# Jackz915/PackPPI

Hardware: AMD Instinct MI355X
Metric: sampled residues/sec at 100 diffusion steps (higher is better)
Workload: dtype f32 (dense layers as split-f16: two f16 per operand, three f16 MFMAs per product, fp32 accumulate); 1 GPU; data/T1124_lig.pdb (L=739, 738 true residues), 1 complex per GPU; diffusion_steps=100, proximal=False, residues_per_gpu=738, residues_rank0=738, residues_total=738, mode=ode

## Files before the change

### packppi_amd/csrc/pp_api.hip

```cpp
#include <math.h>
#include <stdio.h>
#include <stdlib.h>
#include <string.h>

#include <new>
#include <string>
#include <vector>

#include "pp_internal.h"
#include "pp_topk_aten.h"
#include <algorithm>
#include <cstring>
#include <cmath>
#include <chrono>

static thread_local std::string g_err;
void pp_set_error(const std::string &msg) { g_err = msg; }

extern "C" const char *pp_last_error(void) { return g_err.c_str(); }
extern "C" int pp_version(void) { return 101; }
#ifndef PP_BUILD_ID
#define PP_BUILD_ID "unstamped-unstamped"
#endif
static const char g_build_id[] = "PP_BUILD_ID=" PP_BUILD_ID;
// ... 526 lines not shown
extern "C" void pp_ctx_destroy(pp_ctx *c) {
    if (!c) return;
    if (c->arena) {
        pp_plan *p = c->plan;
        std::lock_guard<std::mutex> g(p->pool_mutex);
        if (p->arena_pool.size() < 4) {
            p->arena_pool.push_back({c->arena, c->arena_bytes, c->last_stream});
        } else {
            (void)hipFree(c->arena);
        }
    }
    for (hipEvent_t e : c->prof_ev) (void)hipEventDestroy(e);
    delete c;
}

__global__ void k_fill_seg(int2 *__restrict__ seg, int N, int L) {
    const int n = blockIdx.x * blockDim.x + threadIdx.x;
    if (n < N) seg[n] = make_int2((n / L) * L, L);
}
__global__ void k_fill_seg_packed(int2 *__restrict__ seg, int N, const int32_t *__restrict__ off, int n_seg, int max_len) {
    const int n = blockIdx.x * blockDim.x + threadIdx.x;
    if (n >= N) return;
    int lo = 0, hi = n_seg - 1;
    while (lo < hi) {
        const int mid = (lo + hi + 1) >> 1;
        if (off[mid] <= n) lo = mid; else hi = mid - 1;
    }
    int start = off[lo], len = off[lo + 1] - off[lo];
    start = start < 0 ? 0 : (start > n ? n : start);
    len = len > max_len ? max_len : len;
// ... 78 lines not shown
        char *base = static_cast<char *>(c->arena);
        for (const Slot &sl : slots) { *sl.p = base; base += sl.bytes; }
    }
    if (st == PP_OK) {
        hipStream_t s_ = static_cast<hipStream_t>(stream);
        if (packed) hipLaunchKernelGGL(k_fill_seg_packed, dim3((c->N + 255) / 256), dim3(256), 0, s_, c->seg, c->N, seg_offsets, n_seg, c->L);
        else hipLaunchKernelGGL(k_fill_seg, dim3((c->N + 255) / 256), dim3(256), 0, s_, c->seg, c->N, c->L);
        if (hipGetLastError() != hipSuccess) { pp_set_error("segment table launch failed"); st = PP_ERR_HIP; }
    }
    if (st == PP_OK && hipMemsetAsync(c->sat, 0, 4 * sizeof(unsigned), static_cast<hipStream_t>(stream)) != hipSuccess) {
        pp_set_error("clearing the saturation word failed");
        st = PP_ERR_HIP;
    }
    if (net && st == PP_OK) flag_nonfinite(c, c->b.X, 42, 12, static_cast<hipStream_t>(stream));
    if (net && st == PP_OK) st = pp_launch_prepare(c, static_cast<hipStream_t>(stream));
    if (net && st == PP_OK) st = pp_launch_edge_static(c, static_cast<hipStream_t>(stream));
    if (st != PP_OK) { pp_ctx_destroy(c); return st; }
    *out = c;
    return PP_OK;
}

extern "C" pp_status pp_complex_prepare(pp_plan *plan, const pp_batch *b, void *stream, pp_ctx **out) {
    return prepare_impl(plan, b, nullptr, 0, 0, 0, stream, out);
}

extern "C" pp_status pp_complex_prepare_packed(pp_plan *plan, const pp_batch *b, const int32_t *seg_offsets, int n_seg,
                                               int min_len, int max_len, void *stream, pp_ctx **out) {
    if (!seg_offsets) FAIL(PP_ERR_INVALID, "pp_complex_prepare_packed: null segment offsets");
    return prepare_impl(plan, b, seg_offsets, n_seg, min_len, max_len, stream, out);
}
// ... 73 lines not shown
                             const StepParams *cur, const StepParams *next) {
    pp_status st;
    for (int l = 0; l < 3; l++) {
        if (l == 0 || !pp_edge_fused()) {
            prof_arm(c, 0);
            st = pp_launch_node_message(c, l, s);
            prof_disarm(c);
            if (st != PP_OK) return st;
        }
        if (l < 2) {
            prof_arm(c, 2);
            st = pp_launch_node_update(c, l, PP_NU_MID, chi, step, mode, noise, nullptr, nullptr, s);
            prof_disarm(c);
            if (st != PP_OK) return st;
            prof_arm(c, 1);
            st = pp_launch_edge_update(c, l, s);
            prof_disarm(c);
            if (st != PP_OK) return st;
        } else {
            prof_arm(c, 2);
            st = pp_launch_node_update(c, l, last_mode, chi, step, mode, noise, cur, last_mode == PP_NU_STEP ? next : nullptr, s);
            prof_disarm(c);
            if (st != PP_OK) return st;
        }
    }
    return PP_OK;
}

extern "C" pp_status pp_score(pp_ctx *c, const float *chi, float t, float *score, float *hV, void *stream) {
    if (c) c->last_stream = static_cast<hipStream_t>(stream);
    if (!c || !chi || !score) FAIL(PP_ERR_INVALID, "pp_score: null argument");
// ... 169 lines not shown
```

### packppi_amd/csrc/pp_edge.hip

```cpp
#include "pp_internal.h"

unsigned int pp_edge_range_hits(int) { return 0; }

typedef float f32x16 __attribute__((ext_vector_type(16)));
typedef float f32x4v __attribute__((ext_vector_type(4)));

#define ET 256
#define CH32 (128 * 32)
#define XBUF_FLOATS (4 * 4 * 64 * 4)
#define PARAM_FLOATS 1152

#define MFMA(a, b, c) __builtin_amdgcn_mfma_f32_32x32x2f32((a), (b), (c), 0, 0, 0)

struct EdgeArgs {
    int N, K;
    float inv_K;
    const float *rmask;
    const int32_t *eidx;
    const float *mask_att;
    const float *frames;
    const float *pts;
    const float *PA, *PC;
    const float *hE_in;
    float *hE_out;
// ... 288 lines not shown
    WSTAGE(C0 + 11 + 8 * (c) + 6, NCH, xbuf_get(xbuf, 2, lane, acc); mfma_tile32<false>(wslot, acc, out, lane))   \
    WSTAGE(C0 + 11 + 8 * (c) + 7, NCH, xbuf_get(xbuf, 3, lane, acc); mfma_tile32<false>(wslot, acc, out, lane))

template <int S, bool ST0, bool FUSE>
__global__ void __launch_bounds__(ET, PP_EU_WGS)
k_edge_update(EdgeArgs A) {
    extern __shared__ __attribute__((aligned(16))) float smem[];
    float *xbuf = smem + 4 * S * 1024, *prm = xbuf + XBUF_FLOATS;
    const int tid = threadIdx.x, lane = tid & 63;
    const int wave = __builtin_amdgcn_readfirstlane(tid >> 6);
    const int j = lane & 31, h = lane >> 5;
    const int n = blockIdx.x;
    const int K = A.K;
    const int jj = j < K ? j : K - 1;
    if (A.rmask[n] == 0.f) {
        if (j < K) {
            f32x4v z = {0.f, 0.f, 0.f, 0.f};
            float *orow = A.hE_out + ((size_t)n * K + j) * 128 + 32 * wave;
#pragma unroll
            for (int q = 0; q < 4; q++) *reinterpret_cast<f32x4v *>(orow + 8 * q + 4 * h) = z;
        }
        if constexpr (FUSE) {
            if (tid < 128) A.S[(size_t)n * 128 + tid] = 0.f;
            if (tid == 0) A.msum[n] = 0.f;
        }
        return;
    }
    constexpr int C0 = ST0 ? 0 : 4;
    constexpr int NEU = C0 + 43;
    constexpr int NCH = NEU + (FUSE ? 11 : 0);
    PROLOGUE_PIPE()
// ... 71 lines not shown
    else if (wave == 1) { _Pragma("unroll") for (int r = 0; r < 16; r++) out[r] += x[1][r]; }
    else if (wave == 2) { _Pragma("unroll") for (int r = 0; r < 16; r++) out[r] += x[2][r]; }
    else { _Pragma("unroll") for (int r = 0; r < 16; r++) out[r] += x[3][r]; }
    __syncthreads();
    xbuf_put(xbuf, wave, lane, out);
    __syncthreads();
#pragma unroll
    for (int t = 0; t < 4; t++) xbuf_get(xbuf, t, lane, x[t]);
    float mean3;
    const float rstd = ln_center(x, mean3);
#pragma unroll
    for (int r = 0; r < 16; r++) out[r] -= mean3;
    ln_affine_tile(out, rstd, A.g3 + 32 * wave, A.be3 + 32 * wave, h);
#pragma unroll
    for (int r = 0; r < 16; r++) out[r] *= me;
    store_tile(A.hE_out + ((size_t)n * K + jj) * 128 + 32 * wave, h, out);
    if constexpr (FUSE) {
        int o_pts = n * 48, o_fr = n * 12, o_pa = n * 128;
        int o_ptsj = nbr * 48, o_pc = nbr * 128;
        __syncthreads();
        xbuf_put(xbuf, wave, lane, out);
        asm volatile("" : "+s"(o_pts), "+s"(o_fr), "+s"(o_pa), "+v"(o_ptsj), "+v"(o_pc) : : "memory");
        edge_geometry(A.pts2 + o_pts, A.frames + o_fr, A.pts2 + o_ptsj, h, g);
        load_tile(A.PA2 + o_pa + 32 * wave, h, acc);
        add_tile(A.PC2 + o_pc + 32 * wave, h, acc);
        const float bmid = A.b_mid2[32 * wave + j];
        __builtin_amdgcn_sched_barrier(0);
        __syncthreads();
#pragma unroll
        for (int t = 0; t < 4; t++) xbuf_get(xbuf, t, lane, x[t]);
        WSTAGE(NEU + 0, NCH, mfma_tile32<false>(wslot, x[0], acc, lane))
// ... 111 lines not shown
}

void pp_edge_occupancy(int *node_msg, int *edge_upd) {
    edge_attrs();
    (void)hipOccupancyMaxActiveBlocksPerMultiprocessor(node_msg, reinterpret_cast<const void *>(k_node_message<PP_NM_SLOTS, false>), ET, NM_SMEM);
    (void)hipOccupancyMaxActiveBlocksPerMultiprocessor(edge_upd, reinterpret_cast<const void *>(k_edge_update<PP_EU_SLOTS, false, true>), ET, EU_SMEM);
}

#define EDGE_ATTR_CHECK()                                                                                   \
    if (!edge_attrs()) {                                                                                    \
        pp_set_error("hipFuncSetAttribute(MaxDynamicSharedMemorySize) failed for the edge kernels");        \
        return PP_ERR_HIP;                                                                                  \
    }

extern "C" int pp_edge_variant(void) { return 0; }
bool pp_edge_fused() { return true; }

pp_status pp_launch_edge_static(pp_ctx *c, hipStream_t s) {
    EDGE_ATTR_CHECK()
    EdgeArgs A = edge_args(c, 0, false);
    A.wstream = c->plan->static_stream;
    hipLaunchKernelGGL(k_edge_static<2>, dim3(c->N), dim3(ET), ST_SMEM, s, A);
    PP_HIP_CHECK(hipGetLastError());
    return PP_OK;
}

pp_status pp_launch_node_message(pp_ctx *c, int layer, hipStream_t s) {
    EDGE_ATTR_CHECK()
    EdgeArgs A = edge_args(c, layer, false);
    if (layer == 0) PP_LAUNCH(c, (k_node_message<PP_NM_SLOTS, true>), dim3(c->N), dim3(ET), NM_SMEM, s, A);
    else PP_LAUNCH(c, (k_node_message<PP_NM_SLOTS, false>), dim3(c->N), dim3(ET), NM_SMEM, s, A);
    PP_HIP_CHECK(hipGetLastError());
    return PP_OK;
}

pp_status pp_launch_edge_update(pp_ctx *c, int layer, hipStream_t s) {
    EDGE_ATTR_CHECK()
    if (layer < 0 || layer > 1) { pp_set_error("pp_launch_edge_update: layer must be 0 or 1"); return PP_ERR_INVALID; }
    EdgeArgs A = edge_args(c, layer, true);
    if (layer == 0) PP_LAUNCH(c, (k_edge_update<PP_EU_SLOTS, true, true>), dim3(c->N), dim3(ET), EU_SMEM, s, A);
    else PP_LAUNCH(c, (k_edge_update<PP_EU_SLOTS, false, true>), dim3(c->N), dim3(ET), EU_SMEM, s, A);
    PP_HIP_CHECK(hipGetLastError());
    return PP_OK;
}
```

### packppi_amd/csrc/pp_edge_f16.hip

```cpp
#include "pp_internal.h"

PP_RANGE_COUNTER
PP_RANGE_READER(pp_edge_range_hits)

typedef float f32x16 __attribute__((ext_vector_type(16)));
typedef float f32x4v __attribute__((ext_vector_type(4)));
typedef _Float16 h8 __attribute__((ext_vector_type(8)));

struct HT {
    h8 hi[2], lo[2];
};
typedef float f32x2v __attribute__((ext_vector_type(2)));
typedef _Float16 h2v __attribute__((ext_vector_type(2)));
typedef __fp16 fp16x2_t __attribute__((ext_vector_type(2)));
__device__ __forceinline__ h2v cvt2(f32x2v x) {
    const fp16x2_t r = __builtin_amdgcn_cvt_pkrtz(x[0], x[1]);
    return __builtin_bit_cast(h2v, r);
}
__device__ __forceinline__ f32x2v split_residual(h2v hh, f32x2v x) {
    const unsigned hp = __builtin_bit_cast(unsigned, hh);
    float d0, d1;
    asm("v_fma_mix_f32 %0, %1, -1.0, %2 op_sel_hi:[1,0,0]" : "=v"(d0) : "v"(hp), "v"(x[0]));
    asm("v_fma_mix_f32 %0, %1, -1.0, %2 op_sel:[1,0,0] op_sel_hi:[1,0,0]" : "=v"(d1) : "v"(hp), "v"(x[1]));
    return f32x2v{d0, d1};
// ... 51 lines not shown
    const float *hE_in;
    float *hE_out;
    float *S, *msum;
    const float *wstream;
    const float *params;
    const float *g3, *be3;
    const float *b_mid;
    const float *Z;
    const float *pts2, *PA2, *PC2, *b_mid2;
    float *Znm, *Zem;
    const float *ls_in, *ls_x1, *ls_out;
    unsigned *sat;
    float *dbg;
    int n_pairs;
    int mix_mode;
};
enum { P_BMID = 0, P_BOUT = 128, P_FOB = 256, P_G2 = 384, P_BE2 = 512, P_FIB = 640 };

#ifndef PP_WDEPTH
#define PP_WDEPTH 2
#endif
#ifndef PP_WDEPTH_R1
#define PP_WDEPTH_R1 2
#endif
#define WDEPTH_ (R == 1 ? PP_WDEPTH_R1 : PP_WDEPTH)
#if defined(PP_X_TS) && defined(PP_X_TS_FINE)
#define TSF(k) if constexpr ((k) >= PP_X_TS_FINE && (k) < PP_X_TS_FINE + 16) tsf[(k) - PP_X_TS_FINE] = (int)(__builtin_readcyclecounter() - ts0f);
#else
#define TSF(k)
#endif
// ... 447 lines not shown
        if (live[r]) {
            if (h == 0) A.S[(size_t)n[r] * 128 + 32 * wave + j] = s * A.inv_K;
            if (tid == 0) A.msum[n[r]] = ms * A.inv_K;
        }
    }
    if (pp_sat_hit(sat)) atomicOr(A.sat, 1u);
}

#ifndef PP_NM_WGS2
#define PP_NM_WGS2 3
#endif
template <int R, bool ST0>
__global__ void __launch_bounds__(ET, R == 1 ? PP_WGS : PP_NM_WGS2)
k_node_message(EdgeArgs A) {
    extern __shared__ __attribute__((aligned(16))) float smem[];
    node_message_body<R, ST0>(A, blockIdx.x * R, smem);
}

#define FFN_BIAS_FETCH(c) load_tile(A.params + P_FIB + 128 * (c) + 32 * wave, h, fib);
#define FFN_BLOCK(c)                                                                                         \
    _Pragma("unroll") for (int r = 0; r < R; r++) acc[r] = fib;                                              \
    if constexpr ((c) == 0) { RLAYER_OWN(C0 + 11 + 8 * (c), NCH, acc, x1buf, false, false) }                 \
    else { RLAYER_BUF(C0 + 11 + 8 * (c), NCH, acc, x1buf, false, true) }                                     \
    PUBLISH_OWN(true, acc, xbuf)                                                                             \
    if constexpr ((c) < 3) { FFN_BIAS_FETCH((c) + 1) }                                                       \
    RLAYER_OWN(C0 + 11 + 8 * (c) + 4, NCH, out, xbuf, false, false)

#ifdef PP_X_TS
#define TS(i) { tsv[i] = (int)(__builtin_readcyclecounter() - ts0); }
#else
#define TS(i)
#endif
template <int R, bool ST0, bool FUSE, bool LNS = false>
__device__ __forceinline__ void edge_update_body(const EdgeArgs &A, const int res0, float *smem) {
    float *const xbuf = smem, *const x1buf = smem + R * XBUF_FLOATS, *const stat = x1buf + R * XBUF_FLOATS,
                 *const prm = stat + R * STAT_FLOATS;
    const int tid = threadIdx.x, lane = tid & 63;
    const int wave = __builtin_amdgcn_readfirstlane(tid >> 6);
    const int j = lane & 31, h = lane >> 5;
    const int K = A.K;
    const int jj = j < K ? j : K - 1;
    unsigned sat = 0;
    GROUP_SETUP()
#pragma unroll
    for (int r = 0; r < R; r++)
        if (inr[r] && !live[r]) {
            if (j < K) {
                f32x4v z = {0.f, 0.f, 0.f, 0.f};
                float *orow = A.hE_out + ((size_t)n[r] * K + j) * 128 + 32 * wave;
#pragma unroll
                for (int q = 0; q < 4; q++) *reinterpret_cast<f32x4v *>(orow + 8 * q + 4 * h) = z;
            }
            if constexpr (FUSE) {
                if (tid < 128) A.S[(size_t)n[r] * 128 + tid] = 0.f;
                if (tid == 0) A.msum[n[r]] = 0.f;
            }
        }
    if (first < 0) return;
#pragma unroll
    for (int r = 0; r < R; r++)
        if (!live[r]) n[r] = first;
    constexpr int C0 = ST0 ? 0 : 4;
// ... 98 lines not shown
    FFN_BLOCK(3)
    TS(10)
#pragma unroll
    for (int r = 0; r < R; r++) ln_partial(out[r], stat + r * STAT_FLOATS, wave, j, h);
    __syncthreads();
    TS(11)
#pragma unroll
    for (int r = 0; r < R; r++) {
        float mean3;
        const float rstd = ln_merge(stat + r * STAT_FLOATS, j, mean3);
#pragma unroll
        for (int q = 0; q < 16; q++) out[r][q] -= mean3;
        ln_affine_tile(out[r], rstd, prm + PARAM_LDS + 32 * wave, prm + PARAM_LDS + 128 + 32 * wave, h);
#pragma unroll
        for (int q = 0; q < 16; q++) out[r][q] *= me[r];
        if (live[r]) store_tile(A.hE_out + ((size_t)n[r] * K + jj) * 128 + 32 * wave, h, out[r]);
    }
    TS(12)
    if constexpr (FUSE) {
        GeoI gi_[R];
        float pj2[R][3];
#pragma unroll
        for (int r = 0; r < R; r++) {
            asm volatile("" : "+v"(nbr[r]));
            geo_load_i(A.pts2 + (size_t)n[r] * 48, A.frames + (size_t)n[r] * 12, h, wave, gi_[r]);
            geo_load_j(A.pts2 + (size_t)nbr[r] * 48, h, wave, pj2[r]);
            load_tile(A.PA2 + (size_t)n[r] * 128 + 32 * wave, h, acc[r]);
        }
        __builtin_amdgcn_sched_barrier(0);
        PUBLISH_OPERAND(out, xbuf, A.ls_out)
        __builtin_amdgcn_sched_barrier(0);
// ... 52 lines not shown
    TS(17)
    if (A.dbg && tid == 0)
        for (int q = 0; q < 18; q++) A.dbg[(size_t)n[0] * 24 + q] = (float)tsv[q];
    if (A.dbg && tid == 0) A.dbg[(size_t)n[0] * 24 + 18] = (float)((ts0 >> 6) & 0xFFFFF);
#ifdef PP_X_TS_FINE
    if (A.dbg && tid == 0)
        for (int q = 0; q < 16; q++) A.dbg[(size_t)n[0] * 24 + q] = (float)tsf[q];
#endif
#endif
}

template <int R, bool ST0, bool FUSE, bool LNS = false>
__global__ void __launch_bounds__(ET, R == 1 ? PP_WGS : PP_WGS2)
k_edge_update(EdgeArgs A) {
    extern __shared__ __attribute__((aligned(16))) float smem[];
    edge_update_body<R, ST0, FUSE, LNS>(A, blockIdx.x * R, smem);
}

template <bool ST0, bool FUSE, bool LNS = false>
__global__ void __launch_bounds__(ET, 2)
k_edge_update_mix(EdgeArgs A) {
    extern __shared__ __attribute__((aligned(16))) float smem[];
    const int b = blockIdx.x;
    int pair = -1, single = -1;
    if (A.mix_mode == 2) {
        const int ns = gridDim.x - A.n_pairs;
        if (b < 2 * ns) { if (b & 1) single = b >> 1; else pair = b >> 1; }
        else pair = b - ns;
    } else if (A.mix_mode == 3) {
        const int ns = gridDim.x - A.n_pairs;
        if (b < ns) single = b; else pair = b - ns;
    } else {
        if (b < A.n_pairs) pair = b; else single = b - A.n_pairs;
    }
    if (pair >= 0) edge_update_body<2, ST0, FUSE, LNS>(A, 2 * pair, smem);
    else edge_update_body<1, ST0, FUSE, LNS>(A, 2 * A.n_pairs + single, smem);
}

template <bool ST0>
__global__ void __launch_bounds__(ET, 2)
k_node_message_mix(EdgeArgs A) {
    extern __shared__ __attribute__((aligned(16))) float smem[];
    const int b = blockIdx.x;
    const int ns = gridDim.x - A.n_pairs;
    if (b < ns) node_message_body<1, ST0>(A, 2 * A.n_pairs + b, smem);
    else node_message_body<2, ST0>(A, 2 * (b - ns), smem);
}

template <bool LNS>
__global__ void __launch_bounds__(ET, 1)
k_edge_static(EdgeArgs A) {
    extern __shared__ __attribute__((aligned(16))) float smem[];
    constexpr int R = 1;
    const int tid = threadIdx.x, lane = tid & 63;
    const int wave = __builtin_amdgcn_readfirstlane(tid >> 6);
    const int j = lane & 31, h = lane >> 5;
    const int n = blockIdx.x;
    const int K = A.K;
// ... 170 lines not shown
    PP_HIP_CHECK(hipGetLastError());
    return PP_OK;
}

static float *g_dbg = nullptr;
#ifdef PP_DIAG
extern "C" void pp_debug_set_dbg(float *p) { g_dbg = p; }
#endif
static EdgeArgs edge_args(pp_ctx *c, int layer, bool edge) {
    const pp_plan *p = c->plan;
    const LayerOff &o = p->off.layer[layer];
    EdgeArgs A;
    A.N = c->N; A.K = c->K; A.inv_K = 1.0f / (float)c->K;
    A.n_pairs = 0;
    A.mix_mode = 0;
    A.rmask = c->b.residue_mask;
    A.eidx = c->eidx; A.mask_att = c->mask_att; A.frames = c->frames;
    A.pts = edge ? c->ptsE : c->ptsN;
    A.PA = edge ? c->PAe : c->PAn;
    A.PC = edge ? c->PCe : c->PCn;
    A.hE_in = layer == 0 ? c->hE0 : c->hE;
    A.hE_out = c->hE;
    A.S = c->S; A.msum = c->msum;
    A.wstream = edge ? p->lt[layer].em_stream : p->lt[layer].nm_stream;
    A.params = p->lt[layer].em_params;
    A.g3 = p->w + o.norm_g[3]; A.be3 = p->w + o.norm_b[3];
    A.b_mid = p->w + o.nm_mid_b;
    A.Z = edge ? c->Zem : c->Znm;
    A.Znm = c->Znm; A.Zem = c->Zem;
    A.pts2 = c->ptsN; A.PA2 = c->PAn; A.PC2 = c->PCn;
// ... 89 lines not shown
    }
    if (g_forced_R >= 1 && g_forced_R <= PP_RMAX) return g_forced_R;
    return N > PP_WGS * g_num_cu ? 2 : 1;
}

static int g_mix = -1;
static bool use_mix(int N) {
    if (g_mix < 0) {
        const char *e = PP_GETENV("PP_EDGE_MIX");
        g_mix = e ? atoi(e) : 3;
    }
    if (g_forced_R >= 1 || !g_mix) return false;
    return N > 2 * g_num_cu && N <= 3 * g_num_cu;
}

void pp_edge_occupancy(int *node_msg, int *edge_upd) {
    edge_attrs();
    (void)hipOccupancyMaxActiveBlocksPerMultiprocessor(node_msg, reinterpret_cast<const void *>(nm_kernel_r(1, false)), ET, nm_smem(1));
    (void)hipOccupancyMaxActiveBlocksPerMultiprocessor(edge_upd, reinterpret_cast<const void *>(eu_kernel_r(1, false)), ET, eu_smem(1));
}

#define EDGE_ATTR_CHECK()                                                                                   \
    if (!edge_attrs()) {                                                                                    \
        pp_set_error("hipFuncSetAttribute(MaxDynamicSharedMemorySize) failed for the edge kernels");        \
        return PP_ERR_HIP;                                                                                  \
    }

pp_status pp_launch_edge_static(pp_ctx *c, hipStream_t s) {
    EDGE_ATTR_CHECK()
    EdgeArgs A = edge_args(c, 0, false);
// ... 3 lines not shown
    PP_HIP_CHECK(hipGetLastError());
    return PP_OK;
}

pp_status pp_launch_node_message(pp_ctx *c, int layer, hipStream_t s) {
    EDGE_ATTR_CHECK()
    EdgeArgs A = edge_args(c, layer, false);
    static const char *nm_env = PP_GETENV("PP_NM_R");
    static const int nm_R = nm_env ? atoi(nm_env) : 0;
    const int R = (nm_R >= 1 && nm_R <= PP_RMAX) ? nm_R : pick_R(c->N);
    static const char *nmix_env = PP_GETENV("PP_NM_MIX");
    static const bool nmix = !(nmix_env && atoi(nmix_env) == 0);
    if (nmix && !(nm_R >= 1 && nm_R <= PP_RMAX) && use_mix(c->N)) {
        A.n_pairs = (c->N + 2) / 3;
        const int singles = c->N - 2 * A.n_pairs > 0 ? c->N - 2 * A.n_pairs : 0;
        PP_LAUNCH(c, (layer == 0 ? k_node_message_mix<true> : k_node_message_mix<false>), dim3(A.n_pairs + singles), dim3(ET),
                  nm_smem(2), s, A);
        PP_HIP_CHECK(hipGetLastError());
        return PP_OK;
    }
    PP_LAUNCH(c, nm_kernel_r(R, layer == 0), dim3((c->N + R - 1) / R), dim3(ET), nm_smem(R), s, A);
    PP_HIP_CHECK(hipGetLastError());
    return PP_OK;
}

extern "C" int pp_edge_variant(void) { return 1; }
bool pp_edge_fused() { return PP_FUSED; }

pp_status pp_launch_edge_update(pp_ctx *c, int layer, hipStream_t s) {
    EDGE_ATTR_CHECK()
    if (layer < 0 || layer > 1) { pp_set_error("pp_launch_edge_update: layer must be 0 or 1"); return PP_ERR_INVALID; }
    EdgeArgs A = edge_args(c, layer, true);
    const int R = pick_R(c->N);
    const bool lns = c->plan->ln_scale != nullptr;
    if (lns && !PP_FUSED) { pp_set_error("pp_launch_edge_update: a plan with LayerNorm operand scales needs the fused build"); return PP_ERR_UNSUPPORTED; }
    if (use_mix(c->N)) {
        A.n_pairs = (c->N + 2) / 3;
        A.mix_mode = g_mix;
        const int singles = c->N - 2 * A.n_pairs > 0 ? c->N - 2 * A.n_pairs : 0;
        PP_LAUNCH(c, mix_kernel(layer == 0, lns), dim3(A.n_pairs + singles), dim3(ET), eu_smem(2) > eu_smem(1) ? eu_smem(2) : eu_smem(1), s, A);
        PP_HIP_CHECK(hipGetLastError());
        return PP_OK;
    }
    PP_LAUNCH(c, eu_kernel_r(R, layer == 0, lns), dim3((c->N + R - 1) / R), dim3(ET), eu_smem(R), s, A);
    PP_HIP_CHECK(hipGetLastError());
    return PP_OK;
}
```

### packppi_amd/csrc/pp_internal.h

```cpp
#pragma once
#include <hip/hip_runtime.h>
#include <hip/hip_ext.h>
#include <vector>
#include <mutex>
#include <stdint.h>
#include <string>

#include "../../include/packppi_hip.h"

#if defined(PP_LAB) && !defined(PP_DIAG)
#define PP_DIAG
#endif
#if !defined(PP_LAB) &&                                                                                                       \
    (defined(PP_X_TS) || defined(PP_X_TS_FINE) || defined(PP_X_NOWLOAD) || defined(PP_X_E_NOMFMA) || defined(PP_X_NOSAT) ||      \
     defined(PP_WDEPTH) || defined(PP_WDEPTH_R1) || defined(PP_NXB_R1) || defined(PP_WGS2) || defined(PP_WGS) ||                 \
     defined(PP_NM_WGS2) ||                                                                                                  \
     defined(PP_LDS_PAD) || defined(PP_NO_FUSE_NM) || defined(PP_NU_DEPTH))
#error "PP_X_* / tuning switches compile laboratory variants (most give wrong results): add -DPP_LAB and build a TAGGED library (python -m packppi_amd.build --tag NAME -DPP_LAB -DPP_X_...)"
#endif
#ifdef PP_DIAG
#define PP_GETENV(name) getenv(name)
#else
#define PP_GETENV(name) ((const char *)nullptr)
#endif
// ... 62 lines not shown
    float *side_extent;
    float *bounds_lower, *bounds_upper;
    float clash_tol;
    bool clash_params_set;
};

struct StepParams {
    float temb[16];
    float c_ode;
    float w;
    float c_drift;
    float c_diff;
    float pad[12];
};

struct pp_ctx {
    pp_plan *plan;
    pp_batch b;
    int B, L, K, N;
    bool packed = false;
    int2 *seg;
    int32_t *eidx;
    float *mask_att;
    float *frames;
    float *bbpos;
    float *hE0;
    float *Znm, *Zem;
    float *hE;
    float *hV;
    float *hV_alt;
    float *S;
    float *msum;
    float *ptsN, *PAn, *PCn;
    float *ptsE, *PAe, *PCe;
    float *score;
    float *chi_tmp;
    void *arena = nullptr;
// ... 100 lines not shown
    const float ang = sgn * acosf(pp_dot_t(n1, n2));
    return (ang != ang) ? 0.f : ang;
}
#endif

pp_status pp_launch_prepare(pp_ctx *c, hipStream_t s, const int64_t *E_idx = nullptr);
pp_status pp_launch_node_embed(pp_ctx *c, const float *chi, const StepParams &sp, hipStream_t s);
pp_status pp_launch_node_update(pp_ctx *c, int layer, int last_mode, float *chi, int step, int mode,
                                const float *noise, const StepParams *cur, const StepParams *next, hipStream_t s);
pp_status pp_launch_edge_static(pp_ctx *c, hipStream_t s);
#ifdef PP_EDGE_F16
pp_status pp_launch_edge_embed_f16(pp_ctx *c, hipStream_t s);
#endif
pp_status pp_launch_node_message(pp_ctx *c, int layer, hipStream_t s);
bool pp_edge_fused();
pp_status pp_launch_edge_update(pp_ctx *c, int layer, hipStream_t s);
pp_status pp_launch_atom14(pp_ctx *c, const float *chi, float *xyz, hipStream_t s);
pp_status pp_launch_clash(pp_ctx *c, const float *xyz, float *per_res, float *dchi, hipStream_t s, bool use_candidates = false);
pp_status pp_launch_proximal(pp_ctx *c, const float *chi, float lamda, int nsteps, float *traj,
                             float *chi_last, float *losses, hipStream_t s);

void pp_edge_occupancy(int *node_msg, int *edge_upd);

#define PP_NU_MID 0
#define PP_NU_SCORE 1
#define PP_NU_STEP 2
```

### packppi_amd/csrc/pp_node.hip

```cpp
#include <string.h>

#include "pp_internal.h"
#include <utility>

PP_RANGE_COUNTER
PP_RANGE_READER(pp_node_range_hits)

#define NT 512
#ifndef PP_NODE_GROUPS
#define PP_NODE_GROUPS 1
#endif
#define NG PP_NODE_GROUPS
#define NB (4 * NG)

struct NodeArgs {
    int N;
    const float *rmask;
    const int64_t *rtype;
    const float *bb_sincos;
    const float *sc_mask;
    const uint8_t *m1pi, *m2pi;
    const float *frames;
    const float *embT, *emb_b, *emb_g, *emb_beta;
    float *hV, *S, *msum;
// ... 258 lines not shown
struct NUpdArgs {
    int N;
    const float *rmask;
    const int64_t *rtype;
    const float *bb_sincos;
    const float *sc_mask;
    const uint8_t *m1pi, *m2pi;
    const float *frames;
    const float *embT;
    const float *wstream, *params;
    const float *hV;
    float *hV_out;
    const float *S, *msum;
    float *ptsN, *PAn, *PCn, *ptsE, *PAe, *PCe, *score;
    unsigned *sat;
};

template <bool LAST>
__device__ constexpr int nu_slot_waves(int s) {
    if (!LAST) return s < 52 ? 8 : 3;
    return s < 36 ? 8 : s < 40 ? 4 : s < 46 ? 1 : s < 55 ? 8 : 2;
}

template <int CL>
__device__ __forceinline__ int nu_phys_slot(int s, int q) {
    if constexpr (CL == 1) return s;
    constexpr int NPS = 16 / CL;
    return s < 36 ? s : s < 36 + NPS ? s + NPS * q : s + (16 - NPS);
}
template <bool LAST, int CL>
// ... 102 lines not shown
    _Pragma("unroll") for (int ks_ = 0; ks_ < 4; ks_++) ldB(HI, LO, r * NU_S128 + 8 * g, ks_, bh[ks_], bl[ks_]);
#define FOSTAGE(s)                                                                                   \
    NSTAGE(20 + (s), cH, {                                                                           \
        if constexpr ((s) + 1 < 16) ldB(sm.c_hi, sm.c_lo, r * NU_S512 + 8 * g, (s) + 1, fh[((s) + 1) & 1], fl[((s) + 1) & 1]); \
        mm3(AK, fh[(s) & 1], fl[(s) & 1], cH, cL);                                                   \
    })

template <int MODE, int NU_ND, int CL = 1>
__global__ void __launch_bounds__(512)
k_node_update(NUpdArgs A, float *chi, int step, int sde, const float *noise, int embed_next, StepScalars sp, TimeEmb te_next) {
    static_assert(CL == 1 || MODE == PP_NU_MID, "only the middle layers have a split form");
    constexpr int NU_NRING = NU_ND + 1;
    constexpr bool LAST = MODE != PP_NU_MID;
    constexpr int NSLOT = LAST ? PP_NU_SLOTS_LAST : PP_NU_SLOTS_MID;
    constexpr int NLOAD = MODE == PP_NU_SCORE ? 46 : CL > 1 ? 36 + 16 / CL + 4 : NSLOT;
    const int clq = CL > 1 ? (int)(blockIdx.x % CL) : 0;
    constexpr int NPAR = LAST ? NU_P_LAST_TOTAL : NU_P_MID_TOTAL;
    extern __shared__ __attribute__((aligned(16))) char smem_raw[];
    SmemU &sm = *reinterpret_cast<SmemU *>(smem_raw);
    const int tid = threadIdx.x, lane = tid & 63, wv = __builtin_amdgcn_readfirstlane(tid >> 6);
    const int r = lane & 15, g = lane >> 4, N = A.N, n0 = (int)(blockIdx.x / CL) * 16;
    const int n = n0 + r, nc = n < N ? n : N - 1;
    const bool live = n < N;
    const int fc = 16 * wv + 4 * g;
    const float *par = sm.par;

    const int srow = tid >> 5, scol = (tid & 31) * 4, sn = n0 + srow < N ? n0 + srow : N - 1;
    const nf4 s4 = *reinterpret_cast<const nf4 *>(A.S + (size_t)sn * 128 + scol);
    const nf4 hv4 = *reinterpret_cast<const nf4 *>(A.hV + (size_t)nc * 128 + fc);
    const float ms = A.msum[nc], rm = A.rmask[nc];
    const nf4 zero4i = {0.f, 0.f, 0.f, 0.f};
    float chi1 = 0.f, scm1 = 0.f, nz1 = 0.f, nz2 = 0.f;
    unsigned char m1raw = 0, m2raw = 0;
    int rt = 0;
    nf4 spv = zero4i;
    if constexpr (MODE == PP_NU_STEP) {
// ... 661 lines not shown
    A.rmask = c->b.residue_mask;
    A.rtype = c->b.residue_type;
    A.bb_sincos = c->b.BB_D_sincos;
    A.sc_mask = c->b.SC_D_mask;
    A.m1pi = c->b.chi_1pi_periodic_mask;
    A.m2pi = c->b.chi_2pi_periodic_mask;
    A.frames = c->frames;
    A.embT = p->node_emb_T;
    A.wstream = t.nu_stream;
    A.params = t.nu_params;
    A.hV = c->hV; A.hV_out = c->hV; A.S = c->S; A.msum = c->msum;
    A.ptsN = c->ptsN; A.PAn = c->PAn; A.PCn = c->PCn;
    A.ptsE = c->ptsE; A.PAe = c->PAe; A.PCe = c->PCe;
    A.score = c->score;
    A.sat = c->sat;
    int embed_next = (last_mode == PP_NU_STEP && embed_next_step) ? 1 : 0;
    const dim3 grid((c->N + 15) / 16), block(512);
    const int sde = mode == PP_MODE_SDE ? 1 : 0;
    StepScalars sp = {0.f, 0.f, 0.f, 0.f};
    TimeEmb te = {};
    if (cur) sp = {cur->c_ode, cur->w, cur->c_drift, cur->c_diff};
    if (next) memcpy(te.v, next->temb, sizeof(te.v));
#ifndef PP_EDGE_F16
    {
        static const bool f16_node = PP_GETENV("PP_NODE_F16") != nullptr;
        if (!f16_node) {
            const LayerOff &o = p->off.layer[layer];
            NodeArgs NA = make_args(c);
            UpdW W;
            W.outT = t.nm_out_T; W.out_b = p->w + o.nm_out_b;
// ... 16 lines not shown
            else
                PP_LAUNCH(c, k_node_update_valu<PP_NU_SCORE>, vgrid, vblock, sizeof(Smem), s, NA, W, chi, step, sde, noise, embed_next, pre0, sp, te);
            PP_HIP_CHECK(hipGetLastError());
            return PP_OK;
        }
    }
#endif
    const bool multi = (int)grid.x > g_nu_cus;
    static const char *split_env = PP_GETENV("PP_NU_SPLIT");
    static const int split_max = split_env ? atoi(split_env) : 4;
    const int tiles = (int)grid.x;
    const int cl = last_mode != PP_NU_MID ? 1 : (split_max >= 4 && 4 * tiles <= g_nu_cus) ? 4 : (split_max >= 2 && 2 * tiles <= g_nu_cus) ? 2 : 1;
    if (cl > 1) {
        A.hV_out = c->hV_alt;
        std::swap(c->hV, c->hV_alt);
        PP_LAUNCH(c, nu_kernel_split(cl), dim3(tiles * cl), block, sizeof(SmemU), s, A, chi, step, sde, noise, embed_next, sp, te);
        PP_HIP_CHECK(hipGetLastError());
        return PP_OK;
    }
    const nu_kernel_t kern = nu_kernel(last_mode == PP_NU_MID ? 0 : last_mode == PP_NU_STEP ? 1 : 2, multi);
    PP_LAUNCH(c, kern, grid, block, sizeof(SmemU), s, A, chi, step, sde, noise, embed_next, sp, te);
    PP_HIP_CHECK(hipGetLastError());
    return PP_OK;
}
```

Baseline: 61660 residues/s.

## Map residue blocks to XCDs for neighbour locality and skip dead hE store

Adds an XCD-aware block-to-work mapping so that contiguous residue ranges (and their mostly local kNN neighbours) are processed on the same XCD of the MI355X. The node-message, edge-update and node-update kernels all use it, with the aim of improving L2 hit rates for neighbour gathers. Separately, the last layer's edge update in STEP mode no longer writes hE_out, because that output is unused, which saves global stores. The remapping relies on round-robin dispatch of blocks to XCDs and can leave some blocks idle through early returns.

```diff
diff --git a/packppi_amd/csrc/pp_api.hip b/packppi_amd/csrc/pp_api.hip
--- a/packppi_amd/csrc/pp_api.hip
+++ b/packppi_amd/csrc/pp_api.hip
@@ -564,6 +564,19 @@
     delete c;
 }
 
+static void xcd_report(pp_ctx *c, hipStream_t s) {
+    std::vector<int32_t> e((size_t)c->N * c->K);
+    if (hipStreamSynchronize(s) != hipSuccess ||
+        hipMemcpy(e.data(), c->eidx, e.size() * sizeof(int32_t), hipMemcpyDeviceToHost) != hipSuccess) return;
+    std::vector<int> cls(c->N, 0);
+    for (int i = 0; i < 16; i++)
+        for (int r = pp_xcd_bnd(c->xmap, i); r < pp_xcd_bnd(c->xmap, i + 1) && r < c->N; r++) cls[r] = i & 7;
+    size_t same = 0;
+    for (size_t q = 0; q < e.size(); q++) same += (unsigned)e[q] < (unsigned)c->N && cls[q / c->K] == cls[e[q]];
+    fprintf(stderr, "[pp] XCD map: N %d, %d pairs + %d items of %d, %.1f %% of the %zu neighbour pairs on one XCD\n", c->N, c->xmap.P,
+            c->xmap.S, c->xmap.Rs, 100.0 * same / (double)e.size(), e.size());
+}
+
 __global__ void k_fill_seg(int2 *__restrict__ seg, int N, int L) {
     const int n = blockIdx.x * blockDim.x + threadIdx.x;
     if (n < N) seg[n] = make_int2((n / L) * L, L);
@@ -672,6 +685,8 @@
     }
     if (net && st == PP_OK) flag_nonfinite(c, c->b.X, 42, 12, static_cast<hipStream_t>(stream));
     if (net && st == PP_OK) st = pp_launch_prepare(c, static_cast<hipStream_t>(stream));
+    if (net) c->xmap = pp_edge_xcd_map(c->N);
+    if (net && st == PP_OK && c->xmap.on && PP_GETENV("PP_DEBUG")) xcd_report(c, static_cast<hipStream_t>(stream));
     if (net && st == PP_OK) st = pp_launch_edge_static(c, static_cast<hipStream_t>(stream));
     if (st != PP_OK) { pp_ctx_destroy(c); return st; }
     *out = c;
@@ -775,7 +790,7 @@
             prof_disarm(c);
             if (st != PP_OK) return st;
             prof_arm(c, 1);
-            st = pp_launch_edge_update(c, l, s);
+            st = pp_launch_edge_update(c, l, s, l == 0 || last_mode != PP_NU_STEP);
             prof_disarm(c);
             if (st != PP_OK) return st;
         } else {
diff --git a/packppi_amd/csrc/pp_edge.hip b/packppi_amd/csrc/pp_edge.hip
--- a/packppi_amd/csrc/pp_edge.hip
+++ b/packppi_amd/csrc/pp_edge.hip
@@ -326,7 +326,7 @@
     const int K = A.K;
     const int jj = j < K ? j : K - 1;
     if (A.rmask[n] == 0.f) {
-        if (j < K) {
+        if (j < K && A.hE_out) {
             f32x4v z = {0.f, 0.f, 0.f, 0.f};
             float *orow = A.hE_out + ((size_t)n * K + j) * 128 + 32 * wave;
 #pragma unroll
@@ -428,7 +428,7 @@
     ln_affine_tile(out, rstd, A.g3 + 32 * wave, A.be3 + 32 * wave, h);
 #pragma unroll
     for (int r = 0; r < 16; r++) out[r] *= me;
-    store_tile(A.hE_out + ((size_t)n * K + jj) * 128 + 32 * wave, h, out);
+    if (A.hE_out) store_tile(A.hE_out + ((size_t)n * K + jj) * 128 + 32 * wave, h, out);
     if constexpr (FUSE) {
         int o_pts = n * 48, o_fr = n * 12, o_pa = n * 128;
         int o_ptsj = nbr * 48, o_pc = nbr * 128;
@@ -570,6 +570,7 @@
     }
 
 extern "C" int pp_edge_variant(void) { return 0; }
+PPXcd pp_edge_xcd_map(int) { return PPXcd{}; }
 bool pp_edge_fused() { return true; }
 
 pp_status pp_launch_edge_static(pp_ctx *c, hipStream_t s) {
@@ -590,10 +591,11 @@
     return PP_OK;
 }
 
-pp_status pp_launch_edge_update(pp_ctx *c, int layer, hipStream_t s) {
+pp_status pp_launch_edge_update(pp_ctx *c, int layer, hipStream_t s, bool store_hE) {
     EDGE_ATTR_CHECK()
     if (layer < 0 || layer > 1) { pp_set_error("pp_launch_edge_update: layer must be 0 or 1"); return PP_ERR_INVALID; }
     EdgeArgs A = edge_args(c, layer, true);
+    if (!store_hE) A.hE_out = nullptr;
     if (layer == 0) PP_LAUNCH(c, (k_edge_update<PP_EU_SLOTS, true, true>), dim3(c->N), dim3(ET), EU_SMEM, s, A);
     else PP_LAUNCH(c, (k_edge_update<PP_EU_SLOTS, false, true>), dim3(c->N), dim3(ET), EU_SMEM, s, A);
     PP_HIP_CHECK(hipGetLastError());
diff --git a/packppi_amd/csrc/pp_edge_f16.hip b/packppi_amd/csrc/pp_edge_f16.hip
--- a/packppi_amd/csrc/pp_edge_f16.hip
+++ b/packppi_amd/csrc/pp_edge_f16.hip
@@ -89,6 +89,7 @@
     float *dbg;
     int n_pairs;
     int mix_mode;
+    PPXcd xm;
 };
 enum { P_BMID = 0, P_BOUT = 128, P_FOB = 256, P_G2 = 384, P_BE2 = 512, P_FIB = 640 };
 
@@ -566,7 +567,9 @@
 __global__ void __launch_bounds__(ET, R == 1 ? PP_WGS : PP_NM_WGS2)
 k_node_message(EdgeArgs A) {
     extern __shared__ __attribute__((aligned(16))) float smem[];
-    node_message_body<R, ST0>(A, blockIdx.x * R, smem);
+    const int item = pp_xcd_item(A.xm, (int)blockIdx.x, 0);
+    if (item < 0) return;
+    node_message_body<R, ST0>(A, item * R, smem);
 }
 
 #define FFN_BIAS_FETCH(c) load_tile(A.params + P_FIB + 128 * (c) + 32 * wave, h, fib);
@@ -597,7 +600,7 @@
 #pragma unroll
     for (int r = 0; r < R; r++)
         if (inr[r] && !live[r]) {
-            if (j < K) {
+            if (j < K && A.hE_out) {
                 f32x4v z = {0.f, 0.f, 0.f, 0.f};
                 float *orow = A.hE_out + ((size_t)n[r] * K + j) * 128 + 32 * wave;
 #pragma unroll
@@ -726,7 +729,7 @@
         ln_affine_tile(out[r], rstd, prm + PARAM_LDS + 32 * wave, prm + PARAM_LDS + 128 + 32 * wave, h);
 #pragma unroll
         for (int q = 0; q < 16; q++) out[r][q] *= me[r];
-        if (live[r]) store_tile(A.hE_out + ((size_t)n[r] * K + jj) * 128 + 32 * wave, h, out[r]);
+        if (live[r] && A.hE_out) store_tile(A.hE_out + ((size_t)n[r] * K + jj) * 128 + 32 * wave, h, out[r]);
     }
     TS(12)
     if constexpr (FUSE) {
@@ -809,7 +812,9 @@
 __global__ void __launch_bounds__(ET, R == 1 ? PP_WGS : PP_WGS2)
 k_edge_update(EdgeArgs A) {
     extern __shared__ __attribute__((aligned(16))) float smem[];
-    edge_update_body<R, ST0, FUSE, LNS>(A, blockIdx.x * R, smem);
+    const int item = pp_xcd_item(A.xm, (int)blockIdx.x, 0);
+    if (item < 0) return;
+    edge_update_body<R, ST0, FUSE, LNS>(A, item * R, smem);
 }
 
 template <bool ST0, bool FUSE, bool LNS = false>
@@ -818,7 +823,11 @@
     extern __shared__ __attribute__((aligned(16))) float smem[];
     const int b = blockIdx.x;
     int pair = -1, single = -1;
-    if (A.mix_mode == 2) {
+    if (A.xm.on) {
+        const int item = pp_xcd_item(A.xm, b, 0);
+        if (item < 0) return;
+        if (item < A.n_pairs) pair = item; else single = item - A.n_pairs;
+    } else if (A.mix_mode == 2) {
         const int ns = gridDim.x - A.n_pairs;
         if (b < 2 * ns) { if (b & 1) single = b >> 1; else pair = b >> 1; }
         else pair = b - ns;
@@ -837,6 +846,13 @@
 k_node_message_mix(EdgeArgs A) {
     extern __shared__ __attribute__((aligned(16))) float smem[];
     const int b = blockIdx.x;
+    if (A.xm.on) {
+        const int item = pp_xcd_item(A.xm, b, 0);
+        if (item < 0) return;
+        if (item < A.n_pairs) node_message_body<2, ST0>(A, 2 * item, smem);
+        else node_message_body<1, ST0>(A, A.n_pairs + item, smem);
+        return;
+    }
     const int ns = gridDim.x - A.n_pairs;
     if (b < ns) node_message_body<1, ST0>(A, 2 * A.n_pairs + b, smem);
     else node_message_body<2, ST0>(A, 2 * (b - ns), smem);
@@ -1037,6 +1053,7 @@
     A.N = c->N; A.K = c->K; A.inv_K = 1.0f / (float)c->K;
     A.n_pairs = 0;
     A.mix_mode = 0;
+    A.xm = PPXcd{};
     A.rmask = c->b.residue_mask;
     A.eidx = c->eidx; A.mask_att = c->mask_att; A.frames = c->frames;
     A.pts = edge ? c->ptsE : c->ptsN;
@@ -1156,6 +1173,22 @@
     return N > 2 * g_num_cu && N <= 3 * g_num_cu;
 }
 
+PPXcd pp_edge_xcd_map(int N) {
+    static const char *env = PP_GETENV("PP_XCD_MAP");
+    static const bool on = !(env && atoi(env) == 0);
+    PPXcd m = {};
+    if (!on || !edge_attrs()) return m;
+    const int R = pick_R(N);
+    m.on = 1; m.N = N;
+    if (use_mix(N)) {
+        if (g_mix != 3) return PPXcd{};
+        m.P = (N + 2) / 3; m.S = N - 2 * m.P > 0 ? N - 2 * m.P : 0; m.Rs = 1;
+    } else {
+        m.P = 0; m.S = (N + R - 1) / R; m.Rs = R;
+    }
+    return m;
+}
+
 void pp_edge_occupancy(int *node_msg, int *edge_upd) {
     edge_attrs();
     (void)hipOccupancyMaxActiveBlocksPerMultiprocessor(node_msg, reinterpret_cast<const void *>(nm_kernel_r(1, false)), ET, nm_smem(1));
@@ -1189,12 +1222,14 @@
     if (nmix && !(nm_R >= 1 && nm_R <= PP_RMAX) && use_mix(c->N)) {
         A.n_pairs = (c->N + 2) / 3;
         const int singles = c->N - 2 * A.n_pairs > 0 ? c->N - 2 * A.n_pairs : 0;
-        PP_LAUNCH(c, (layer == 0 ? k_node_message_mix<true> : k_node_message_mix<false>), dim3(A.n_pairs + singles), dim3(ET),
-                  nm_smem(2), s, A);
+        if (c->xmap.on && c->xmap.P == A.n_pairs) A.xm = c->xmap;
+        PP_LAUNCH(c, (layer == 0 ? k_node_message_mix<true> : k_node_message_mix<false>),
+                  dim3(A.xm.on ? pp_xcd_grid(A.xm, 0) : A.n_pairs + singles), dim3(ET), nm_smem(2), s, A);
         PP_HIP_CHECK(hipGetLastError());
         return PP_OK;
     }
-    PP_LAUNCH(c, nm_kernel_r(R, layer == 0), dim3((c->N + R - 1) / R), dim3(ET), nm_smem(R), s, A);
+    if (c->xmap.on && c->xmap.P == 0 && c->xmap.Rs == R) A.xm = c->xmap;
+    PP_LAUNCH(c, nm_kernel_r(R, layer == 0), dim3(A.xm.on ? pp_xcd_grid(A.xm, 0) : (c->N + R - 1) / R), dim3(ET), nm_smem(R), s, A);
     PP_HIP_CHECK(hipGetLastError());
     return PP_OK;
 }
@@ -1202,10 +1237,11 @@
 extern "C" int pp_edge_variant(void) { return 1; }
 bool pp_edge_fused() { return PP_FUSED; }
 
-pp_status pp_launch_edge_update(pp_ctx *c, int layer, hipStream_t s) {
+pp_status pp_launch_edge_update(pp_ctx *c, int layer, hipStream_t s, bool store_hE) {
     EDGE_ATTR_CHECK()
     if (layer < 0 || layer > 1) { pp_set_error("pp_launch_edge_update: layer must be 0 or 1"); return PP_ERR_INVALID; }
     EdgeArgs A = edge_args(c, layer, true);
+    if (!store_hE && PP_FUSED) A.hE_out = nullptr;
     const int R = pick_R(c->N);
     const bool lns = c->plan->ln_scale != nullptr;
     if (lns && !PP_FUSED) { pp_set_error("pp_launch_edge_update: a plan with LayerNorm operand scales needs the fused build"); return PP_ERR_UNSUPPORTED; }
@@ -1213,11 +1249,14 @@
         A.n_pairs = (c->N + 2) / 3;
         A.mix_mode = g_mix;
         const int singles = c->N - 2 * A.n_pairs > 0 ? c->N - 2 * A.n_pairs : 0;
-        PP_LAUNCH(c, mix_kernel(layer == 0, lns), dim3(A.n_pairs + singles), dim3(ET), eu_smem(2) > eu_smem(1) ? eu_smem(2) : eu_smem(1), s, A);
+        if (c->xmap.on && c->xmap.P == A.n_pairs && g_mix == 3) A.xm = c->xmap;
+        PP_LAUNCH(c, mix_kernel(layer == 0, lns), dim3(A.xm.on ? pp_xcd_grid(A.xm, 0) : A.n_pairs + singles), dim3(ET),
+                  eu_smem(2) > eu_smem(1) ? eu_smem(2) : eu_smem(1), s, A);
         PP_HIP_CHECK(hipGetLastError());
         return PP_OK;
     }
-    PP_LAUNCH(c, eu_kernel_r(R, layer == 0, lns), dim3((c->N + R - 1) / R), dim3(ET), eu_smem(R), s, A);
+    if (c->xmap.on && c->xmap.P == 0 && c->xmap.Rs == R) A.xm = c->xmap;
+    PP_LAUNCH(c, eu_kernel_r(R, layer == 0, lns), dim3(A.xm.on ? pp_xcd_grid(A.xm, 0) : (c->N + R - 1) / R), dim3(ET), eu_smem(R), s, A);
     PP_HIP_CHECK(hipGetLastError());
     return PP_OK;
 }
diff --git a/packppi_amd/csrc/pp_internal.h b/packppi_amd/csrc/pp_internal.h
--- a/packppi_amd/csrc/pp_internal.h
+++ b/packppi_amd/csrc/pp_internal.h
@@ -100,6 +100,39 @@
     float pad[12];
 };
 
+struct PPXcd {
+    int on;
+    int N, P, S, Rs;
+};
+__host__ __device__ __forceinline__ int pp_xcd_bnd(const PPXcd &m, int i) {
+    if (i <= 8) return 2 * ((m.P * i) >> 3);
+    const int r = 2 * m.P + m.Rs * ((m.S * (i - 8)) >> 3);
+    return r < m.N ? r : m.N;
+}
+__host__ __device__ __forceinline__ int pp_xcd_first(const PPXcd &m, int i, int cl) {
+    if (cl == 0) return i <= 8 ? (m.P * i) >> 3 : m.P + ((m.S * (i - 8)) >> 3);
+    const int T = (m.N + 15) >> 4;
+    if (i >= 16) return cl * T;
+    const int t = (pp_xcd_bnd(m, i) + 7) >> 4;
+    return cl * (t < T ? t : T);
+}
+__host__ __device__ __forceinline__ int pp_xcd_item(const PPXcd &m, int b, int cl) {
+    if (!m.on) return b;
+    const int x = b & 7, k = b >> 3;
+    const int s1 = pp_xcd_first(m, x + 8, cl), n1 = pp_xcd_first(m, x + 9, cl) - s1;
+    if (k < n1) return s1 + k;
+    const int s0 = pp_xcd_first(m, x, cl), n0 = pp_xcd_first(m, x + 1, cl) - s0;
+    return k - n1 < n0 ? s0 + k - n1 : -1;
+}
+inline int pp_xcd_grid(const PPXcd &m, int cl) {
+    int mx = 0;
+    for (int x = 0; x < 8; x++) {
+        const int n = pp_xcd_first(m, x + 1, cl) - pp_xcd_first(m, x, cl) + pp_xcd_first(m, x + 9, cl) - pp_xcd_first(m, x + 8, cl);
+        mx = n > mx ? n : mx;
+    }
+    return 8 * mx;
+}
+
 struct pp_ctx {
     pp_plan *plan;
     pp_batch b;
@@ -107,6 +140,7 @@
     bool packed = false;
     int2 *seg;
     int32_t *eidx;
+    PPXcd xmap = {};
     float *mask_att;
     float *frames;
     float *bbpos;
@@ -237,13 +271,14 @@
 #endif
 pp_status pp_launch_node_message(pp_ctx *c, int layer, hipStream_t s);
 bool pp_edge_fused();
-pp_status pp_launch_edge_update(pp_ctx *c, int layer, hipStream_t s);
+pp_status pp_launch_edge_update(pp_ctx *c, int layer, hipStream_t s, bool store_hE = true);
 pp_status pp_launch_atom14(pp_ctx *c, const float *chi, float *xyz, hipStream_t s);
 pp_status pp_launch_clash(pp_ctx *c, const float *xyz, float *per_res, float *dchi, hipStream_t s, bool use_candidates = false);
 pp_status pp_launch_proximal(pp_ctx *c, const float *chi, float lamda, int nsteps, float *traj,
                              float *chi_last, float *losses, hipStream_t s);
 
 void pp_edge_occupancy(int *node_msg, int *edge_upd);
+PPXcd pp_edge_xcd_map(int N);
 
 #define PP_NU_MID 0
 #define PP_NU_SCORE 1
diff --git a/packppi_amd/csrc/pp_node.hip b/packppi_amd/csrc/pp_node.hip
--- a/packppi_amd/csrc/pp_node.hip
+++ b/packppi_amd/csrc/pp_node.hip
@@ -296,6 +296,7 @@
     const float *S, *msum;
     float *ptsN, *PAn, *PCn, *ptsE, *PAe, *PCe, *score;
     unsigned *sat;
+    PPXcd xm;
 };
 
 template <bool LAST>
@@ -428,12 +429,14 @@
     constexpr bool LAST = MODE != PP_NU_MID;
     constexpr int NSLOT = LAST ? PP_NU_SLOTS_LAST : PP_NU_SLOTS_MID;
     constexpr int NLOAD = MODE == PP_NU_SCORE ? 46 : CL > 1 ? 36 + 16 / CL + 4 : NSLOT;
-    const int clq = CL > 1 ? (int)(blockIdx.x % CL) : 0;
+    const int lb = pp_xcd_item(A.xm, (int)blockIdx.x, CL);
+    if (lb < 0) return;
+    const int clq = CL > 1 ? lb % CL : 0;
     constexpr int NPAR = LAST ? NU_P_LAST_TOTAL : NU_P_MID_TOTAL;
     extern __shared__ __attribute__((aligned(16))) char smem_raw[];
     SmemU &sm = *reinterpret_cast<SmemU *>(smem_raw);
     const int tid = threadIdx.x, lane = tid & 63, wv = __builtin_amdgcn_readfirstlane(tid >> 6);
-    const int r = lane & 15, g = lane >> 4, N = A.N, n0 = (int)(blockIdx.x / CL) * 16;
+    const int r = lane & 15, g = lane >> 4, N = A.N, n0 = (lb / CL) * 16;
     const int n = n0 + r, nc = n < N ? n : N - 1;
     const bool live = n < N;
     const int fc = 16 * wv + 4 * g;
@@ -1125,6 +1128,7 @@
     A.ptsE = c->ptsE; A.PAe = c->PAe; A.PCe = c->PCe;
     A.score = c->score;
     A.sat = c->sat;
+    A.xm = PPXcd{};
     int embed_next = (last_mode == PP_NU_STEP && embed_next_step) ? 1 : 0;
     const dim3 grid((c->N + 15) / 16), block(512);
     const int sde = mode == PP_MODE_SDE ? 1 : 0;
@@ -1171,12 +1175,15 @@
     if (cl > 1) {
         A.hV_out = c->hV_alt;
         std::swap(c->hV, c->hV_alt);
-        PP_LAUNCH(c, nu_kernel_split(cl), dim3(tiles * cl), block, sizeof(SmemU), s, A, chi, step, sde, noise, embed_next, sp, te);
+        const int xg = c->xmap.on ? pp_xcd_grid(c->xmap, cl) : 0;
+        if (xg && xg <= g_nu_cus) A.xm = c->xmap;
+        PP_LAUNCH(c, nu_kernel_split(cl), dim3(A.xm.on ? xg : tiles * cl), block, sizeof(SmemU), s, A, chi, step, sde, noise, embed_next, sp, te);
         PP_HIP_CHECK(hipGetLastError());
         return PP_OK;
     }
     const nu_kernel_t kern = nu_kernel(last_mode == PP_NU_MID ? 0 : last_mode == PP_NU_STEP ? 1 : 2, multi);
-    PP_LAUNCH(c, kern, grid, block, sizeof(SmemU), s, A, chi, step, sde, noise, embed_next, sp, te);
+    A.xm = c->xmap;
+    PP_LAUNCH(c, kern, A.xm.on ? dim3(pp_xcd_grid(A.xm, 1)) : grid, block, sizeof(SmemU), s, A, chi, step, sde, noise, embed_next, sp, te);
     PP_HIP_CHECK(hipGetLastError());
     return PP_OK;
 }
```

Result: no change. 62180 residues/s (median of 6 runs) (+0.8%).
